# angela000/DQNFlappyBird

Measured on NVIDIA B200. Metric: env frames/sec (step+render+preproc), higher is better.
Workload: dtype u8

## Files before the change

dqnflappybird_b200/_lib.py:

```python
from __future__ import annotations

import ctypes as C
import glob
import os
import subprocess

_PKG = os.path.dirname(os.path.abspath(__file__))
_CSRC = os.path.join(_PKG, "csrc")
SO_PATH = os.path.join(_PKG, "libflappy_b200.so")

NVCC_FLAGS = [
    "-gencode", "arch=compute_100a,code=sm_100a", "-lineinfo", "-O3", "-std=c++17",
    "-Xcompiler", "-fPIC", "-shared",
]


class FlappyError(RuntimeError):
    pass


def sources():
    return sorted(glob.glob(os.path.join(_CSRC, "*.cu")))


# ... 117 lines not shown
    "fb_replay_sample_uniform": ([_vp, C.c_longlong, C.c_int, C.c_uint32, C.c_uint64, _i32p, _vp], C.c_int),
    "fb_replay_gather": ([_vp, _u8p, _u8p, _f32p, _u8p, C.c_longlong, C.c_int, _i32p, C.c_int, _u8p, _u8p, _f32p, _u8p, _i32p, _i32p, _vp], C.c_int),
    "fb_per_store": ([_vp, C.c_longlong, C.c_int, _vp], C.c_int),
    "fb_per_sample": ([_vp, C.c_int, C.c_double, C.c_uint64, _i32p, _i32p, _vp, _vp, _f32p, _vp], C.c_int),
    "fb_per_update": ([_vp, _i32p, _f32p, _vp, C.c_int, C.c_int, _vp], C.c_int),
    "fb_per_tree_copy": ([_vp, _vp, C.c_int, _vp], C.c_int),
    "fb_per_aux_tree_copy": ([_vp, C.c_int, _vp, C.c_int, _vp], C.c_int),
    "fb_per_min_root": ([_vp, _vp, _vp], C.c_int),
    "fb_per_set_global_min": ([_vp, _vp], C.c_int),
    "fb_replay_rng_pos": ([_vp, _vp, C.c_int, _vp], C.c_int),
    "fb_debug_assets_load_host": ([C.c_char_p, C.c_size_t], C.c_int),
    "fb_debug_host_reset": ([_i32p, _u8p, C.c_int, C.c_uint64, C.c_uint64], C.c_int),
    "fb_debug_host_step": ([_i32p, C.c_int, _u8p, C.c_int, C.c_uint64, C.c_uint64, _f32p, _u8p, _i32p], C.c_int),
    "fb_debug_host_obs": ([_i32p, C.c_int, _u8p], C.c_int),
    "fb_debug_host_mixed": ([_i32p], C.c_int),
    "fb_debug_tc_mma_rate": ([C.c_int, C.c_int, C.c_int, C.c_int, C.c_int, _vp, _vp], C.c_int),
    "fb_debug_tc_kernel": ([_vp, C.c_int, C.c_int, C.c_int, _f32p, _vp], C.c_int),
    "fb_debug_tc_slab": ([C.c_int, C.c_int, _vp, _vp, _f32p, _vp], C.c_int),
    "fb_debug_tc_gemm": ([C.c_int, C.c_int, C.c_int, C.c_int, C.c_int, _vp, _vp, _f32p, _vp, _vp], C.c_int),
}


def declared_symbols():
    return sorted(_SIGNATURES)


def lib():
    global _lib
    if _lib is None:
        if needs_build():
            build()
# ... 30 lines not shown
```

dqnflappybird_b200/csrc/fb_qnet_tc.cu:

```cuda
#include <cudaTypedefs.h>

#include <stdlib.h>
#include <string.h>

#include <map>
#include <new>
#include <vector>

#include "fb_qnet.cuh"
#include "fb_pack.cuh"
#include "fb_tc.cuh"
#include "fb_tc_conv.cuh"


namespace {

constexpr int kStages = 4;
constexpr int kMaxKb = 32;
constexpr int kG1 = 21, kP1 = 441;
constexpr int kG2 = 7, kP2 = 49;
constexpr int kThreads = 192;

struct GemmParams {
    int nkb, kper;
// ... 1328 lines not shown
    int n_sms;
    cudaStream_t aux;
    cudaStream_t aux2;
    cudaStream_t aux4;
    cudaStream_t aux3;
    cudaStream_t cap;
    cudaEvent_t ev[16];
    std::vector<GraphEntry> graphs;
    int use_graph;
    int f16;
    int fuse_fwd;
    int nopdl;
    int fuse_bwd;
    int step_samples;
    int conv1_mode;
};

namespace {

constexpr int kChunk1 = 1024, kChunk23 = 256;
constexpr int kFc1Splits = 5;
constexpr int kFuseMaxBatch = 512;
bool fused_head_ok(const QnetLayout &L) { return L.hidden == 512; }
int head_ctas(const TcState *t, int B) { const int c = (B + 3) / 4, m = t->n_sms < kMaxHeadCtas ? t->n_sms : kMaxHeadCtas; return c < m ? c : m; }

constexpr int kSlab1 = 152, kSlab2 = 136, kSlab3 = 144;
constexpr int kSlabW1 = 88, kSlabW2 = 72, kSlabW3 = 88;

int plan_splits(long long P, int target, int *klen_out) {
    if (target < 1) target = 1;
// ... 135 lines not shown
    FB_CUDA_OK(cudaDeviceGetAttribute(&t->n_sms, cudaDevAttrMultiProcessorCount, dev));
    {
        int lo = 0, hi = 0;
        FB_CUDA_OK(cudaDeviceGetStreamPriorityRange(&lo, &hi));
        FB_CUDA_OK(cudaStreamCreateWithPriority(&t->aux, cudaStreamNonBlocking, lo));
        FB_CUDA_OK(cudaStreamCreateWithPriority(&t->aux2, cudaStreamNonBlocking, hi));
        FB_CUDA_OK(cudaStreamCreateWithPriority(&t->aux3, cudaStreamNonBlocking, hi));
        FB_CUDA_OK(cudaStreamCreateWithPriority(&t->aux4, cudaStreamNonBlocking, lo));
        FB_CUDA_OK(cudaStreamCreateWithPriority(&t->cap, cudaStreamNonBlocking, hi));
    }
    for (auto &e : t->ev) FB_CUDA_OK(cudaEventCreateWithFlags(&e, cudaEventDisableTiming));
    t->use_graph = 1;
    { const char *e = getenv("FB_TC_FUSE_BWD"); t->fuse_bwd = (e && e[0] == '0') ? 0 : 1; }
    { const char *e = getenv("FB_TC_FUSE_FWD"); t->fuse_fwd = (e && e[0] == '0') ? 0 : 1; }
    { const char *e = getenv("FB_TC_CONV1_MODE"); t->conv1_mode = (e && e[0] >= '0' && e[0] <= '4') ? e[0] - '0' : 4; }
    { const char *e = getenv("FB_TC_NOPDL"); t->nopdl = e ? atoi(e) : 1; }
    n->tc = t;
    return FB_OK;
}

void tc_state_destroy(fb_qnet *n) {
    TcState *t = n->tc;
    if (!t) return;
    for (auto &g : t->graphs) destroy_entry(g);
    for (int w = 0; w < 2; w++) {
        FwdWs &f = t->ws[w];
        void *fs[] = {f.x2, f.z1, f.p2, f.a2, f.a3, f.parth, f.h1};
        for (void *p : fs) cudaFree(p);
    }
    void *ps[] = {t->dh1, t->dz3, t->dz2, t->dp2, t->dz1, t->part1, t->part2, t->part3, t->bp1, t->bp2, t->bp3, t->hp, t->hb, t->loss_terms,
// ... 81 lines not shown
    const QnetLayout &L = n->L;
    const TcWeightMaps &wm = t->wm[slot];
    const FwdWs &f = t->ws[w];
    const int P1 = B * kP1, P2 = B * kP2;
    g_probe_view = fv;
    const int c1mode = conv1_mode_at(t, B);
    if (c1mode == 0) {
        FB_CUDA_OK(tc::launch_pdl(pack_x2_kernel, dim3((unsigned)(((size_t)P1 * 8 + 255) / 256)), dim3(256), 0, st, fv, B, f.x2, t->f16));
        FB_CUDA_OK((launch_tc_conv<32, kSlab1, 1, 4, 6, 1>(p->x2_s[w], wm.w1p, p->conv1, t->n_sms, EpiConv1{f.z1, params_dev + L.b1, P1, t->f16}, st)));
        FB_CUDA_OK(tc::launch_pdl(pool_pack_kernel, dim3((unsigned)(((size_t)B * 36 * 16 + 255) / 256)), dim3(256), 0, st, f.z1, B, f.p2, t->f16));
    } else if ((keep && c1mode != 3) || c1mode == 1) {
        FB_CUDA_OK(tc::launch_pdl(pack_x2_kernel, dim3((unsigned)(((size_t)P1 * 8 + 255) / 256)), dim3(256), 0, st, fv, B, f.x2, t->f16));
        FB_CUDA_OK((launch_tc_conv1_fused<6, true>(p->x2_s[w], wm.w1p, Conv1FusedParams{fv, B, params_dev + L.b1, keep ? f.z1 : nullptr, f.p2, t->f16},
                                                  t->n_sms, st)));
    } else {
        FB_CUDA_OK((launch_tc_conv1_fused<4, false>(p->x2_s[w], wm.w1p, Conv1FusedParams{fv, B, params_dev + L.b1, keep ? f.z1 : nullptr, f.p2, t->f16}, t->n_sms, st)));
    }
    if (t->fuse_fwd && B <= kFuseMaxBatch) {
        FB_CUDA_OK((launch_tc_fwd23<2>(p->p2_s[w], wm.w2p, wm.w3p, Fwd23Params{(B + 1) / 2, B, params_dev + L.b2, params_dev + L.b3, keep ? f.a2 : nullptr, f.a3, t->f16},
                                       t->n_sms, st)));
    } else {
        FB_CUDA_OK((launch_tc_conv<64, kSlab2, 2, 8, 3, 1>(p->p2_s[w], wm.w2p, p->conv2, t->n_sms, EpiGrid7{f.a2, params_dev + L.b2, P2, t->f16}, st)));
        FB_CUDA_OK((launch_tc_conv<64, kSlab3, 1, 9, 4, 1>(p->a2_s[w], wm.w3p, p->conv3, t->n_sms, EpiConv3{f.a3, params_dev + L.b3, P2, t->f16}, st)));
    }
    FB_CUDA_OK((launch_tc_gemm<128, 2>(p->a3_k[w], wm.wf1n, p->fc1, dim3((B + 127) / 128, L.hidden / 128, p->sf),
                                       EpiStoreF32{f.parth, B, L.hidden, (size_t)n->max_batch * L.hidden}, st)));
    if (join) FB_CUDA_OK(cudaStreamWaitEvent(st, join, 0));
    TdFuse none{};
    if (td != nullptr && ap != nullptr && fused_head_ok(L))
        FB_CUDA_OK(tc::launch_pdl(fc1_head_train_kernel<16>, dim3(head_ctas(t, B)), dim3(128), 0, st, f.parth, p->sf,
                                  (size_t)n->max_batch * L.hidden, params_dev, L, B, q_out, *td, HeadBwd{t->dh1, t->hp, t->hb, GradFmt{t->f16, gscale}}, *ap));
// ... 320 lines not shown
    for (int r = 0; r < reps; r++) {
        switch (which) {
            case 0: FB_CUDA_OK((launch_tc_conv<32, kSlab1, 1, 4, 6, 1>(p->x2_s[0], wm.w1p, p->conv1, t->n_sms, EpiConv1{f.z1, params_dev + L.b1, P1, t->f16}, st))); break;
            case 1: FB_CUDA_OK((launch_tc_conv<64, kSlab2, 2, 8, 3, 1>(p->p2_s[0], wm.w2p, p->conv2, t->n_sms, EpiGrid7{f.a2, params_dev + L.b2, P2, t->f16}, st))); break;
            case 2: FB_CUDA_OK((launch_tc_conv<64, kSlab3, 1, 9, 4, 1>(p->a2_s[0], wm.w3p, p->conv3, t->n_sms, EpiConv3{f.a3, params_dev + L.b3, P2, t->f16}, st))); break;
            case 3: FB_CUDA_OK((launch_tc_gemm<128, 2>(p->a3_k[0], wm.wf1n, p->fc1, dim3((B + 127) / 128, H / 128, p->sf),
                                                       EpiStoreF32{f.parth, B, H, (size_t)n->max_batch * H}, st))); break;
            case 4: FB_CUDA_OK((launch_tc_wgrad<32, 2, kSlabW1, 1, 6>(p->x2_w, p->dz1_b, p->conv1_w, p->s1, EpiStoreF32{t->part1, 256, 32, (size_t)256 * 32}, st))); break;
            case 5: FB_CUDA_OK((launch_tc_conv<64, kSlab3, 1, 9, 4, 1>(p->dz3_s, wm.w3d, p->conv3_d, t->n_sms, EpiConv3Dgrad{t->dz2, f.a2, P2, t->f16}, st))); break;
            case 6: FB_CUDA_OK((launch_tc_gemm<64, 0>(p->dh1_k, wm.wf1n, p->fc1_d, dim3((B + 127) / 128, kFlat / 64, 1), EpiFc1Dgrad{t->dz3, f.a3, B, t->f16}, st))); break;
            case 7: FB_CUDA_OK((launch_tc_conv1_fused<4, false>(p->x2_s[0], wm.w1p, Conv1FusedParams{g_probe_view, B, params_dev + L.b1, nullptr, f.p2, t->f16}, t->n_sms, st))); break;
            case 8: FB_CUDA_OK((launch_tc_conv1_fused<4, false>(p->x2_s[0], wm.w1p, Conv1FusedParams{g_probe_view, B, params_dev + L.b1, f.z1, f.p2, t->f16}, t->n_sms, st))); break;
            case 9: FB_CUDA_OK((launch_tc_conv1_fused<6, true>(p->x2_s[0], wm.w1p, Conv1FusedParams{g_probe_view, B, params_dev + L.b1, nullptr, f.p2, t->f16}, t->n_sms, st))); break;
            case 10: FB_CUDA_OK((launch_tc_conv1_fused<6, true>(p->x2_s[0], wm.w1p, Conv1FusedParams{g_probe_view, B, params_dev + L.b1, f.z1, f.p2, t->f16}, t->n_sms, st))); break;
            case 11: FB_CUDA_OK((launch_tc_conv1_fused<6, true>(p->x2_s[0], wm.w1p, Conv1FusedParams{g_probe_view, B, params_dev + L.b1, nullptr, nullptr, t->f16}, t->n_sms, st))); break;
            default: FB_REQUIRE(false, "fb_debug_tc_kernel: which must be 0..11");
        }
    }
    return FB_OK;
}

namespace {
__global__ void __launch_bounds__(128) tc_slab_probe_kernel(const __grid_constant__ CUtensorMap mapA, const __grid_constant__ CUtensorMap mapB,
                                                            int shift, uint32_t base_offset, float *d) {
    extern __shared__ uint8_t smem_raw[];
    __shared__ __align__(8) uint64_t bar_full, bar_done;
    __shared__ uint32_t tmem_slot;
    const uint32_t smem = (tc::smem_u32(smem_raw) + 1023u) & ~1023u;
    const int warp = threadIdx.x >> 5, lane = threadIdx.x & 31;
    if (threadIdx.x == 0) { tc::mbar_init(tc::smem_u32(&bar_full), 1); tc::mbar_init(tc::smem_u32(&bar_done), 1); tc::fence_barrier_init(); }
    if (warp == 0) tc::tmem_alloc(tc::smem_u32(&tmem_slot), 64);
// ... 28 lines not shown

extern "C" int fb_debug_tc_slab(int shift, int base_offset, const void *a_dev, const void *b_dev, float *d_dev, void *stream) {
    FB_REQUIRE(a_dev && b_dev && d_dev && shift >= 0 && shift <= 128, "fb_debug_tc_slab: bad argument");
    int rc = ensure_encode();
    if (rc) return rc;
    CUtensorMap ma, mb;
    if ((rc = make_map(&ma, (const bf16 *)a_dev, 256, 64, 64, 128))) return rc;
    if ((rc = make_map(&mb, (const bf16 *)b_dev, 64, 64, 64, 64))) return rc;
    FB_CUDA_OK(cudaFuncSetAttribute(tc_slab_probe_kernel, cudaFuncAttributeMaxDynamicSharedMemorySize, 32768 + 8192 + 1024));
    tc_slab_probe_kernel<<<1, 128, 32768 + 8192 + 1024, (cudaStream_t)stream>>>(ma, mb, shift, (uint32_t)base_offset, d_dev);
    FB_CUDA_OK(cudaGetLastError());
    return FB_OK;
}

namespace {
__global__ void __launch_bounds__(128) tc_mma_rate_kernel(int n, int mn_major, int naccs, int iters, int same_operands, long long *cycles) {
    extern __shared__ uint8_t smem_raw[];
    __shared__ __align__(8) uint64_t bar;
    __shared__ uint32_t tmem_slot;
    const uint32_t smem = (tc::smem_u32(smem_raw) + 1023u) & ~1023u;
    const int warp = threadIdx.x >> 5;
    for (int i = threadIdx.x; i < 48 * 1024 / 4; i += 128) reinterpret_cast<uint32_t *>(smem_raw)[i] = 0x3c003c00u;
    if (threadIdx.x == 0) { tc::mbar_init(tc::smem_u32(&bar), 1); tc::fence_barrier_init(); }
    if (warp == 0) tc::tmem_alloc(tc::smem_u32(&tmem_slot), 512);
    tc::fence_proxy_async();
    tc::tc_fence_before(); __syncthreads(); tc::tc_fence_after();
    const uint32_t tmem = tmem_slot;
    if (warp == 1) {
        const uint32_t idesc = tc::instr_desc_bf16(128, n, mn_major, mn_major);
        const uint32_t hi = tc::smem_desc_hi(1024, tc::kSwizzle128);
        const uint32_t a0 = tc::smem_desc_lo(smem, mn_major ? 8192 : 16), b0 = tc::smem_desc_lo(smem + 16384, mn_major ? 8192 : 16);
        const uint32_t step = same_operands ? 0 : (mn_major ? 128 : 2);
        const uint32_t d1 = naccs > 1 ? (uint32_t)n : 0, d2 = naccs > 2 ? 2u * n : 0, d3 = naccs > 3 ? 3u * n : d1;
        uint32_t elected;
        asm volatile("{\n\t.reg .pred p;\n\telect.sync _|p, 0xffffffff;\n\tselp.b32 %0, 1, 0, p;\n\t}" : "=r"(elected));
        long long t0 = clock64();
        for (int i = 0; i < iters; i += 8) {
            if (elected) {
                tc::umma_bf16_lohi(tmem, a0, hi, b0, hi, idesc, 1);
                tc::umma_bf16_lohi(tmem + d1, a0 + step, hi, b0 + step, hi, idesc, 1);
                tc::umma_bf16_lohi(tmem + d2, a0 + 2 * step, hi, b0 + 2 * step, hi, idesc, 1);
                tc::umma_bf16_lohi(tmem + d3, a0 + 3 * step, hi, b0 + 3 * step, hi, idesc, 1);
                tc::umma_bf16_lohi(tmem, a0, hi, b0, hi, idesc, 1);
// ... 3 lines not shown
            }
            __syncwarp();
        }
        long long t_issue = clock64();
        if (elected) tc::umma_commit(tc::smem_u32(&bar));
        __syncwarp();
        tc::mbar_wait(tc::smem_u32(&bar), 0);
        long long t1 = clock64();
        if (elected) { cycles[0] = t1 - t0; cycles[1] = t_issue - t0; }
    }
    tc::tc_fence_before(); __syncthreads();
    if (warp == 0) tc::tmem_dealloc(tmem, 512);
}
}

extern "C" int fb_debug_tc_mma_rate(int n, int mn_major, int naccs, int iters, int same_operands, long long *cycles_dev, void *stream) {
    FB_REQUIRE(cycles_dev && n >= 16 && n <= 256 && n % 16 == 0 && naccs >= 1 && naccs * n <= 512 && iters > 0, "fb_debug_tc_mma_rate: bad argument");
    FB_CUDA_OK(cudaFuncSetAttribute(tc_mma_rate_kernel, cudaFuncAttributeMaxDynamicSharedMemorySize, 64 * 1024));
    tc_mma_rate_kernel<<<1, 128, 64 * 1024, (cudaStream_t)stream>>>(n, mn_major, naccs, iters, same_operands, cycles_dev);
    FB_CUDA_OK(cudaGetLastError());
    return FB_OK;
}

extern "C" int fb_debug_tc_gemm(int mode, int bn, int M, int N, int K, const void *a_dev, const void *b_dev, float *d_dev,
                                const uint32_t *strides6, void *stream) {
    FB_REQUIRE(a_dev && b_dev && d_dev && (mode == 0 || mode == 1) && (bn == 32 || bn == 64 || bn == 128) && N % bn == 0,
               "fb_debug_tc_gemm: bad argument");
    int rc = ensure_encode();
    if (rc) return rc;
    cudaStream_t st = (cudaStream_t)stream;
    CUtensorMap ma, mb;
    GemmParams g{};
    const bf16 *A = (const bf16 *)a_dev, *Bm = (const bf16 *)b_dev;
    dim3 grid;
// ... 26 lines not shown
```

dqnflappybird_b200/csrc/fb_tc.cuh:

```cuda
#pragma once
#include <cuda.h>
#include <cuda_bf16.h>
#include <cuda_fp16.h>
#include <cuda_runtime.h>
#include <stdint.h>

namespace tc {

__device__ __forceinline__ uint32_t smem_u32(const void *p) { return (uint32_t)__cvta_generic_to_shared(p); }

__device__ __forceinline__ bool elect_one() {
    uint32_t e;
    asm volatile("{\n\t.reg .pred p;\n\telect.sync _|p, 0xffffffff;\n\tselp.b32 %0, 1, 0, p;\n\t}" : "=r"(e));
    return e != 0;
}

__device__ __forceinline__ void mbar_init(uint32_t bar, uint32_t count) {
    asm volatile("mbarrier.init.shared::cta.b64 [%0], %1;" ::"r"(bar), "r"(count));
}
__device__ __forceinline__ void fence_barrier_init() { asm volatile("fence.mbarrier_init.release.cluster;" ::: "memory"); }
__device__ __forceinline__ void fence_proxy_async() { asm volatile("fence.proxy.async.shared::cta;" ::: "memory"); }
__device__ __forceinline__ void mbar_arrive(uint32_t bar) {
    asm volatile("mbarrier.arrive.shared::cta.b64 _, [%0];" ::"r"(bar) : "memory");
}
// ... 50 lines not shown
        "{\n\t.reg .pred p;\n\t"
        "setp.ne.b32 p, %4, 0;\n\t"
        "tcgen05.mma.cta_group::1.kind::f16 [%0], %1, %2, %3, p;\n\t}"
        ::"r"(d_tmem), "l"(adesc), "l"(bdesc), "r"(idesc), "r"(accumulate)
        : "memory");
}
__device__ __forceinline__ void umma_bf16_lohi(uint32_t d_tmem, uint32_t alo, uint32_t ahi, uint32_t blo, uint32_t bhi, uint32_t idesc,
                                               uint32_t accumulate) {
    asm volatile(
        "{\n\t.reg .pred p;\n\t.reg .b64 da, db;\n\t"
        "mov.b64 da, {%1, %2};\n\t"
        "mov.b64 db, {%3, %4};\n\t"
        "setp.ne.b32 p, %6, 0;\n\t"
        "tcgen05.mma.cta_group::1.kind::f16 [%0], da, db, %5, p;\n\t}"
        ::"r"(d_tmem), "r"(alo), "r"(ahi), "r"(blo), "r"(bhi), "r"(idesc), "r"(accumulate)
        : "memory");
}
__device__ __forceinline__ void umma_commit(uint32_t bar) {
    asm volatile("tcgen05.commit.cta_group::1.mbarrier::arrive::one.shared::cluster.b64 [%0];" ::"r"(bar) : "memory");
}
__device__ __forceinline__ void tmem_ld16(uint32_t taddr, float (&v)[16]) {
    uint32_t r[16];
    asm volatile(
        "tcgen05.ld.sync.aligned.32x32b.x16.b32 {%0,%1,%2,%3,%4,%5,%6,%7,%8,%9,%10,%11,%12,%13,%14,%15}, [%16];"
        : "=r"(r[0]), "=r"(r[1]), "=r"(r[2]), "=r"(r[3]), "=r"(r[4]), "=r"(r[5]), "=r"(r[6]), "=r"(r[7]), "=r"(r[8]),
          "=r"(r[9]), "=r"(r[10]), "=r"(r[11]), "=r"(r[12]), "=r"(r[13]), "=r"(r[14]), "=r"(r[15])
        : "r"(taddr));
    asm volatile("tcgen05.wait::ld.sync.aligned;" ::: "memory");
#pragma unroll
    for (int i = 0; i < 16; i++) v[i] = __uint_as_float(r[i]);
// ... 1 lines not shown

__device__ __forceinline__ void tmem_ld32(uint32_t taddr, float (&v)[32]) {
    uint32_t r[32];
    asm volatile(
        "tcgen05.ld.sync.aligned.32x32b.x32.b32 "
        "{%0,%1,%2,%3,%4,%5,%6,%7,%8,%9,%10,%11,%12,%13,%14,%15,%16,%17,%18,%19,%20,%21,%22,%23,%24,%25,%26,%27,%28,%29,%30,%31}, [%32];"
        : "=r"(r[0]), "=r"(r[1]), "=r"(r[2]), "=r"(r[3]), "=r"(r[4]), "=r"(r[5]), "=r"(r[6]), "=r"(r[7]), "=r"(r[8]), "=r"(r[9]),
          "=r"(r[10]), "=r"(r[11]), "=r"(r[12]), "=r"(r[13]), "=r"(r[14]), "=r"(r[15]), "=r"(r[16]), "=r"(r[17]), "=r"(r[18]), "=r"(r[19]),
          "=r"(r[20]), "=r"(r[21]), "=r"(r[22]), "=r"(r[23]), "=r"(r[24]), "=r"(r[25]), "=r"(r[26]), "=r"(r[27]), "=r"(r[28]), "=r"(r[29]),
          "=r"(r[30]), "=r"(r[31])
        : "r"(taddr));
    asm volatile("tcgen05.wait::ld.sync.aligned;" ::: "memory");
#pragma unroll
    for (int i = 0; i < 32; i++) v[i] = __uint_as_float(r[i]);
}

enum : uint32_t { kSwizzle128 = 2, kSwizzle64 = 4 };
__host__ __device__ constexpr uint64_t smem_desc(uint32_t addr, uint32_t lbo_bytes, uint32_t sbo_bytes, uint32_t layout) {
    return (uint64_t)((addr >> 4) & 0x3FFFu) | ((uint64_t)((lbo_bytes >> 4) & 0x3FFFu) << 16) |
           ((uint64_t)((sbo_bytes >> 4) & 0x3FFFu) << 32) | (1ull << 46) | ((uint64_t)layout << 61);
}
__host__ __device__ constexpr uint32_t smem_desc_lo(uint32_t addr, uint32_t lbo_bytes) {
    return ((addr >> 4) & 0x3FFFu) | (((lbo_bytes >> 4) & 0x3FFFu) << 16);
}
__host__ __device__ constexpr uint32_t smem_desc_hi(uint32_t sbo_bytes, uint32_t layout) {
    return ((sbo_bytes >> 4) & 0x3FFFu) | (1u << 14) | (layout << 29);
}
__host__ __device__ constexpr uint32_t instr_desc_bf16(int m, int n, int a_mn_major, int b_mn_major) {
    return (1u << 4) | (1u << 7) | (1u << 10) | ((uint32_t)a_mn_major << 15) | ((uint32_t)b_mn_major << 16) |
           ((uint32_t)(n >> 3) << 17) | ((uint32_t)(m >> 4) << 24);
// ... 60 lines not shown
```

dqnflappybird_b200/csrc/fb_tc_conv.cuh:

```cuda
#pragma once
#include "fb_tc.cuh"

namespace {

constexpr int kConvThreads = 192;

constexpr size_t kExclusiveSmem = 116 * 1024;
constexpr size_t exclusive_smem(size_t need) { return need > kExclusiveSmem ? need : kExclusiveSmem; }

struct ConvParams {
    int n_tiles;
    int slab_row0;
    int kb_rowoff[16];
    int kb_half[16];
    int f16;
};

template <int BN, int SLAB_ROWS, int NHALF, int NKB, int S, int T, class EP>
__global__ void __launch_bounds__(kConvThreads, 1) tc_conv_kernel(const __grid_constant__ CUtensorMap mapA,
                                                                   const __grid_constant__ CUtensorMap mapB, const ConvParams g, const EP ep) {
    constexpr uint32_t HALF_BYTES = SLAB_ROWS * 128, STAGE = NHALF * HALF_BYTES, BBLK = BN * 128, B_BYTES = NKB * BBLK;
    static_assert(SLAB_ROWS % 8 == 0 && SLAB_ROWS <= 256, "slab rows: multiple of 8 (1024-byte stage alignment), one TMA box");
    static_assert(S % T == 0 && 2 * T * BN <= 512, "a group of T tiles occupies T consecutive stages and T accumulators of a set");
    extern __shared__ uint8_t smem_raw[];
// ... 299 lines not shown
#pragma unroll
    for (int k = 0; k < K; k++) {
        const bool valid = (dst[k] & 0x80000000u) != 0;
        uint32_t w[4];
#pragma unroll
        for (int s2 = 0; s2 < 2; s2++)
#pragma unroll
            for (int h = 0; h < 2; h++) {
                const float lo = (float)((t[k][2 * h] >> (8 * s2)) & 255), hi = (float)((t[k][2 * h + 1] >> (8 * s2)) & 255);
                w[s2 * 2 + h] = valid ? tc::pack2(lo, hi, f16) : 0u;
            }
        if (tid + k * NT <= LAST) *reinterpret_cast<uint4 *>(slab + (dst[k] & 0x7fffffffu)) = make_uint4(w[0], w[1], w[2], w[3]);
    }
}

struct Conv1FusedParams {
    FrameView fv;
    int B;
    const float *bias;
    __nv_bfloat16 *z1;
    __nv_bfloat16 *p2;
    int f16;
};

template <int S, bool FROM_X2>
__global__ void __launch_bounds__(FROM_X2 ? kRoleThreads1 : kFusedThreads, 1) tc_conv1_fused_kernel(const __grid_constant__ CUtensorMap mapA,
                                                                                          const __grid_constant__ CUtensorMap mapB,
                                                                                          const Conv1FusedParams g) {
    constexpr int BN = 32, NKB = 4;
    constexpr uint32_t STAGE = kSlabF * 128, BBLK = BN * 128, B_BYTES = NKB * BBLK, ZS_BYTES = 128 * BN * 2;
    extern __shared__ uint8_t smem_raw[];
    __shared__ __align__(8) uint64_t bar_full[S], bar_empty[S], bar_b, bar_acc_full[2], bar_acc_empty[2], bar_raw_full[kRawStages],
        bar_raw_empty[kRawStages];
    __shared__ uint32_t tmem_slot;
    __shared__ __align__(16) float bias_s[BN];
    uint8_t *smem_gen = smem_raw + ((1024u - (tc::smem_u32(smem_raw) & 1023u)) & 1023u);
    const uint32_t smem_b = tc::smem_u32(smem_gen), smem_a = smem_b + B_BYTES;
    uint8_t *slab_gen = smem_gen + B_BYTES, *zs_gen = slab_gen + S * STAGE, *raw_gen = zs_gen + 4 * ZS_BYTES;
    const int warp = threadIdx.x >> 5, lane = threadIdx.x & 31;
    const int n_tiles = 4 * g.B;
    const long long total_rows = (long long)g.B * 441;

    if (threadIdx.x == 0) {
        tc::tma_prefetch_desc(&mapB);
        for (int s = 0; s < S; s++) { tc::mbar_init(tc::smem_u32(&bar_full[s]), 1); tc::mbar_init(tc::smem_u32(&bar_empty[s]), 1); }
        tc::mbar_init(tc::smem_u32(&bar_b), 1);
        for (int a = 0; a < 2; a++) { tc::mbar_init(tc::smem_u32(&bar_acc_full[a]), 1); tc::mbar_init(tc::smem_u32(&bar_acc_empty[a]), 4); }
        for (int k = 0; k < kRawStages; k++) { tc::mbar_init(tc::smem_u32(&bar_raw_full[k]), 1); tc::mbar_init(tc::smem_u32(&bar_raw_empty[k]), 1); }
        tc::fence_barrier_init();
    }
    if (warp == 1) tc::tmem_alloc(tc::smem_u32(&tmem_slot), 64);
    tc::tc_fence_before();
    __syncthreads();
    tc::tc_fence_after();
    const uint32_t tmem = tmem_slot;
    if (threadIdx.x == 0) {
        tc::mbar_expect_tx(tc::smem_u32(&bar_b), B_BYTES);
        for (int kb = 0; kb < NKB; kb++) tc::tma_load_2d(smem_b + kb * BBLK, &mapB, kb * 64, 0, tc::smem_u32(&bar_b));
    }
    if (threadIdx.x >= 64 && threadIdx.x < 64 + BN) bias_s[threadIdx.x - 64] = g.bias[threadIdx.x - 64];
    tc::pdl_wait();
    tc::pdl_launch();
    __syncthreads();

    if (warp == 0 && FROM_X2) {
        const bool leader = tc::elect_one();
// ... 11 lines not shown
    } else if (warp == 0) {
        const bool leader = tc::elect_one();
        int i = 0;
        for (int tile = blockIdx.x; tile < n_tiles; tile += gridDim.x, i++) {
            const int rs = i % kRawStages, b = tile >> 2, tq = tile & 3;
            tc::mbar_wait(tc::smem_u32(&bar_raw_empty[rs]), ((i / kRawStages) & 1) ^ 1u);
            if (leader) {
                const int ih0 = 24 * tq - 2, lo = ih0 < 0 ? 0 : ih0, hi = ih0 + kRawRows > 80 ? 80 : ih0 + kRawRows;
                const uint32_t bytes = (uint32_t)(hi - lo) * 80u, full = tc::smem_u32(&bar_raw_full[rs]);
                const uint32_t dst = tc::smem_u32(raw_gen) + rs * kRawBytes + (uint32_t)(lo - ih0) * 80u;
                tc::mbar_expect_tx(full, 4 * bytes);
#pragma unroll
                for (int c = 0; c < 4; c++) tc::bulk_load_1d(dst + c * (kRawRows * 80), g.fv.chan(b, c) + lo * 80, bytes, full);
            }
            __syncwarp();
        }
    } else if (warp >= kRoleThreads1 / 32) {
        constexpr int GT = kBuilders / 2;
        const int grp = (threadIdx.x - kRoleThreads1) / GT, tid = (threadIdx.x - kRoleThreads1) - grp * GT;
        int i = grp;
        for (int tile = blockIdx.x + grp * (int)gridDim.x; tile < n_tiles; tile += 2 * (int)gridDim.x, i += 2) {
            const int s = i % S, rs = i % kRawStages;
            tc::mbar_wait(tc::smem_u32(&bar_raw_full[rs]), (i / kRawStages) & 1);
            tc::mbar_wait(tc::smem_u32(&bar_empty[s]), ((i / S) & 1) ^ 1u);
            slab_from_raw<GT>(slab_gen + s * STAGE, raw_gen + rs * kRawBytes, tile & 3, tid, g.f16);
            tc::fence_proxy_async();
            if (grp == 0) asm volatile("bar.sync 2, %0;" ::"n"(GT) : "memory");
            else asm volatile("bar.sync 3, %0;" ::"n"(GT) : "memory");
            if (tid == 0) { tc::mbar_arrive(tc::smem_u32(&bar_full[s])); tc::mbar_arrive(tc::smem_u32(&bar_raw_empty[rs])); }
        }
    } else if (warp == 1) {
        const bool leader = tc::elect_one();
        const uint32_t idesc = tc::instr_desc_16(128, BN, 0, 0, g.f16);
        constexpr uint32_t dhi = tc::smem_desc_hi(1024, tc::kSwizzle128);
        const uint32_t a_lo0 = tc::smem_desc_lo(smem_a, 16), b_lo0 = tc::smem_desc_lo(smem_b, 16);
        tc::mbar_wait(tc::smem_u32(&bar_b), 0);
        int i = 0;
        for (int tile = blockIdx.x; tile < n_tiles; tile += gridDim.x, i++) {
            const int s = i % S, as = i & 1;
            tc::mbar_wait(tc::smem_u32(&bar_acc_empty[as]), ((i >> 1) & 1) ^ 1u);
            tc::mbar_wait(tc::smem_u32(&bar_full[s]), (i / S) & 1);
            tc::tc_fence_after();
            if (leader) {
                const uint32_t a_lo = a_lo0 + s * (STAGE >> 4);
#pragma unroll
                for (int kb = 0; kb < NKB; kb++) {
                    const uint32_t tap = (uint32_t)(((kb >> 1) * 21 + (kb & 1)) * 128) >> 4;
#pragma unroll
                    for (int k = 0; k < 4; k++)
                        tc::umma_bf16_lohi(tmem + as * BN, a_lo + tap + 2 * k, dhi, b_lo0 + ((kb * BBLK + k * 32) >> 4), dhi, idesc, (kb | k) != 0);
                }
                tc::umma_commit(tc::smem_u32(&bar_empty[s]));
                tc::umma_commit(tc::smem_u32(&bar_acc_full[as]));
            }
            __syncwarp();
        }
    } else if (warp >= 2 && warp < kRoleThreads1 / 32) {
        const int eg = (warp - 2) >> 2;
// ... 45 lines not shown
                    const int r0 = (2 * ph_l) * 21 + 2 * pw;
                    uint4 m = ld(r0), o1 = ld(r0 + 1), o2 = ld(r0 + 21), o3 = ld(r0 + 22);
                    uint32_t *pm = reinterpret_cast<uint32_t *>(&m);
                    const uint32_t *p1 = reinterpret_cast<const uint32_t *>(&o1), *p2 = reinterpret_cast<const uint32_t *>(&o2),
                                   *p3 = reinterpret_cast<const uint32_t *>(&o3);
#pragma unroll
                    for (int k = 0; k < 4; k++) pm[k] = tc::max2(tc::max2(pm[k], p1[k], g.f16), tc::max2(p2[k], p3[k], g.f16), g.f16);
                    const int bh = (ph + 1) >> 1, rr = (ph + 1) & 1, bw = (pw + 1) >> 1, ss = (pw + 1) & 1;
                    *reinterpret_cast<uint4 *>(g.p2 + ((size_t)b * 49 + bh * 7 + bw) * 128 + rr * 64 + ss * 32 + cg * 8) = m;
                }
            }
        }
    }
    tc::tc_fence_before();
    __syncthreads();
    if (warp == 1) tc::tmem_dealloc(tmem, 64);
}

template <int S, bool FROM_X2>
static cudaError_t launch_tc_conv1_fused(const CUtensorMap &ma, const CUtensorMap &mb, const Conv1FusedParams &g, int max_ctas, cudaStream_t st) {
    static bool configured = false;
    auto kern = tc_conv1_fused_kernel<S, FROM_X2>;
    constexpr size_t smem = exclusive_smem(4 * 32 * 128 + (size_t)S * kSlabF * 128 + 4 * 128 * 32 * 2 + (FROM_X2 ? 0 : kRawStages * kRawBytes) + 1024);
    if (!configured) {
        cudaError_t e = cudaFuncSetAttribute(kern, cudaFuncAttributeMaxDynamicSharedMemorySize, (int)smem);
        if (e != cudaSuccess) return e;
        configured = true;
    }
    int grid = 4 * g.B < max_ctas ? 4 * g.B : max_ctas;
    return tc::launch_pdl(kern, dim3(grid), dim3(FROM_X2 ? kRoleThreads1 : kFusedThreads), smem, st, ma, mb, g);
}

}
```

include/flappy_b200.h:

```cpp
#ifndef FLAPPY_B200_H
#define FLAPPY_B200_H

#include <stddef.h>
#include <stdint.h>

#ifdef __cplusplus
extern "C" {
#endif

#define FB_OBS 80
#define FB_FRAME_BYTES 6400
#define FB_SCREEN_W 288
#define FB_SCREEN_H 512
#define FB_STATE_INTS 16

typedef enum {
    FB_OK = 0,
    FB_ERR_INVALID = -1,
    FB_ERR_CUDA = -2,
    FB_ERR_ASSETS = -3,
    FB_ERR_ACTION = -4,
    FB_ERR_STATE = -5
} fb_status;

// ... 144 lines not shown
                               const float *target_params_dev, const int32_t *chan_off_s_host4, const int32_t *chan_off_next_host4,
                               int global_batch, double gamma, int loss_sum, float *grads_dev, float *loss_out_dev,
                               float *abs_err_out_dev, float *q_target_out_dev, float *m_dev, float *v_dev, float lr, float beta1,
                               float beta2, float eps, float grad_scale, float beta1_power, float beta2_power, void *stream);


int fb_debug_assets_load_host(const uint8_t *packed_host, size_t n);
int fb_debug_step_sampling_layout(int32_t *out, int capacity);
int fb_debug_host_reset(int32_t *state16, const uint8_t *gaps, int gaps_len, uint64_t seed, uint64_t env_id);
int fb_debug_host_step(int32_t *state16, int action, const uint8_t *gaps, int gaps_len, uint64_t seed,
                       uint64_t env_id, float *reward, uint8_t *terminal, int32_t *score);
int fb_debug_host_obs(const int32_t *state16, int mode , uint8_t *out6400);
int fb_debug_host_mixed(const int32_t *state16);
int fb_debug_tc_gemm(int mode, int bn, int M, int N, int K, const void *a_bf16_dev, const void *b_bf16_dev, float *d_dev,
                     const uint32_t *strides6_host, void *stream);
int fb_debug_tc_mma_rate(int n, int mn_major, int naccs, int iters, int same_operands, long long *cycles_dev, void *stream);
int fb_debug_tc_kernel(fb_qnet *net, int which, int batch, int reps, const float *params_dev, void *stream);
int fb_debug_tc_slab(int shift, int base_offset, const void *a_bf16_dev, const void *b_bf16_dev, float *d_dev, void *stream);

#ifdef __cplusplus
}
#endif
#endif
```

Before: 846.1 million.

## Stage conv1 im2col A operand in tensor memory instead of shared memory

Adds a conv1 fused-kernel variant where builder warps write the im2col A tile straight into tensor memory with tcgen05.st, and the MMA issuer reads A from TMEM. This removes the shared-memory slab for A and the smem writes and reads on that path, at the cost of allocating all 512 TMEM columns and cutting to two pipeline stages. It is on by default in the raw-u8 conv1 mode and can be turned off with an env var. A microbenchmark option for the TMEM-A MMA rate is also added.

```diff
diff --git a/dqnflappybird_b200/_lib.py b/dqnflappybird_b200/_lib.py
--- a/dqnflappybird_b200/_lib.py
+++ b/dqnflappybird_b200/_lib.py
@@ -155,7 +155,7 @@
     "fb_debug_host_step": ([_i32p, C.c_int, _u8p, C.c_int, C.c_uint64, C.c_uint64, _f32p, _u8p, _i32p], C.c_int),
     "fb_debug_host_obs": ([_i32p, C.c_int, _u8p], C.c_int),
     "fb_debug_host_mixed": ([_i32p], C.c_int),
-    "fb_debug_tc_mma_rate": ([C.c_int, C.c_int, C.c_int, C.c_int, C.c_int, _vp, _vp], C.c_int),
+    "fb_debug_tc_mma_rate": ([C.c_int, C.c_int, C.c_int, C.c_int, C.c_int, C.c_int, _vp, _vp], C.c_int),
     "fb_debug_tc_kernel": ([_vp, C.c_int, C.c_int, C.c_int, _f32p, _vp], C.c_int),
     "fb_debug_tc_slab": ([C.c_int, C.c_int, _vp, _vp, _f32p, _vp], C.c_int),
     "fb_debug_tc_gemm": ([C.c_int, C.c_int, C.c_int, C.c_int, C.c_int, _vp, _vp, _f32p, _vp, _vp], C.c_int),
diff --git a/dqnflappybird_b200/csrc/fb_qnet_tc.cu b/dqnflappybird_b200/csrc/fb_qnet_tc.cu
--- a/dqnflappybird_b200/csrc/fb_qnet_tc.cu
+++ b/dqnflappybird_b200/csrc/fb_qnet_tc.cu
@@ -1366,6 +1366,7 @@
     int fuse_bwd;
     int step_samples;
     int conv1_mode;
+    int conv1_tmem;
 };
 
 namespace {
@@ -1531,6 +1532,7 @@
     { const char *e = getenv("FB_TC_FUSE_BWD"); t->fuse_bwd = (e && e[0] == '0') ? 0 : 1; }
     { const char *e = getenv("FB_TC_FUSE_FWD"); t->fuse_fwd = (e && e[0] == '0') ? 0 : 1; }
     { const char *e = getenv("FB_TC_CONV1_MODE"); t->conv1_mode = (e && e[0] >= '0' && e[0] <= '4') ? e[0] - '0' : 4; }
+    { const char *e = getenv("FB_TC_CONV1_TMEM"); t->conv1_tmem = (e && e[0] == '0') ? 0 : 1; }
     { const char *e = getenv("FB_TC_NOPDL"); t->nopdl = e ? atoi(e) : 1; }
     n->tc = t;
     return FB_OK;
@@ -1642,7 +1644,9 @@
         FB_CUDA_OK((launch_tc_conv1_fused<6, true>(p->x2_s[w], wm.w1p, Conv1FusedParams{fv, B, params_dev + L.b1, keep ? f.z1 : nullptr, f.p2, t->f16},
                                                   t->n_sms, st)));
     } else {
-        FB_CUDA_OK((launch_tc_conv1_fused<4, false>(p->x2_s[w], wm.w1p, Conv1FusedParams{fv, B, params_dev + L.b1, keep ? f.z1 : nullptr, f.p2, t->f16}, t->n_sms, st)));
+        const Conv1FusedParams c1{fv, B, params_dev + L.b1, keep ? f.z1 : nullptr, f.p2, t->f16};
+        if (t->conv1_tmem) FB_CUDA_OK((launch_tc_conv1_fused<2, false, true>(p->x2_s[w], wm.w1p, c1, t->n_sms, st)));
+        else FB_CUDA_OK((launch_tc_conv1_fused<4, false>(p->x2_s[w], wm.w1p, c1, t->n_sms, st)));
     }
     if (t->fuse_fwd && B <= kFuseMaxBatch) {
         FB_CUDA_OK((launch_tc_fwd23<2>(p->p2_s[w], wm.w2p, wm.w3p, Fwd23Params{(B + 1) / 2, B, params_dev + L.b2, params_dev + L.b3, keep ? f.a2 : nullptr, f.a3, t->f16},
@@ -1993,7 +1997,9 @@
             case 9: FB_CUDA_OK((launch_tc_conv1_fused<6, true>(p->x2_s[0], wm.w1p, Conv1FusedParams{g_probe_view, B, params_dev + L.b1, nullptr, f.p2, t->f16}, t->n_sms, st))); break;
             case 10: FB_CUDA_OK((launch_tc_conv1_fused<6, true>(p->x2_s[0], wm.w1p, Conv1FusedParams{g_probe_view, B, params_dev + L.b1, f.z1, f.p2, t->f16}, t->n_sms, st))); break;
             case 11: FB_CUDA_OK((launch_tc_conv1_fused<6, true>(p->x2_s[0], wm.w1p, Conv1FusedParams{g_probe_view, B, params_dev + L.b1, nullptr, nullptr, t->f16}, t->n_sms, st))); break;
-            default: FB_REQUIRE(false, "fb_debug_tc_kernel: which must be 0..11");
+            case 12: FB_CUDA_OK((launch_tc_conv1_fused<2, false, true>(p->x2_s[0], wm.w1p, Conv1FusedParams{g_probe_view, B, params_dev + L.b1, nullptr, f.p2, t->f16}, t->n_sms, st))); break;
+            case 13: FB_CUDA_OK((launch_tc_conv1_fused<2, false, true>(p->x2_s[0], wm.w1p, Conv1FusedParams{g_probe_view, B, params_dev + L.b1, f.z1, f.p2, t->f16}, t->n_sms, st))); break;
+            default: FB_REQUIRE(false, "fb_debug_tc_kernel: which must be 0..13");
         }
     }
     return FB_OK;
@@ -2052,7 +2058,8 @@
 }
 
 namespace {
-__global__ void __launch_bounds__(128) tc_mma_rate_kernel(int n, int mn_major, int naccs, int iters, int same_operands, long long *cycles) {
+__global__ void __launch_bounds__(128) tc_mma_rate_kernel(int n, int mn_major, int naccs, int iters, int same_operands, int a_tmem,
+                                                          long long *cycles) {
     extern __shared__ uint8_t smem_raw[];
     __shared__ __align__(8) uint64_t bar;
     __shared__ uint32_t tmem_slot;
@@ -2063,8 +2070,41 @@
     if (warp == 0) tc::tmem_alloc(tc::smem_u32(&tmem_slot), 512);
     tc::fence_proxy_async();
     tc::tc_fence_before(); __syncthreads(); tc::tc_fence_after();
-    const uint32_t tmem = tmem_slot;
-    if (warp == 1) {
+    const uint32_t tmem = tmem_slot, ta = tmem + 480;
+    if (a_tmem) {
+        const uint32_t r[8] = {0x3c003c00u, 0x3c003c00u, 0x3c003c00u, 0x3c003c00u, 0x3c003c00u, 0x3c003c00u, 0x3c003c00u, 0x3c003c00u};
+        for (int c = 0; c < 32; c += 8) tc::tmem_st8(ta + ((uint32_t)(warp * 32) << 16) + (uint32_t)c, r);
+        tc::tmem_st_wait();
+        tc::tc_fence_before(); __syncthreads(); tc::tc_fence_after();
+    }
+    if (warp == 1 && a_tmem) {
+        const uint32_t idesc = tc::instr_desc_bf16(128, n, 0, mn_major);
+        const uint32_t hi = tc::smem_desc_hi(1024, tc::kSwizzle128);
+        const uint32_t b0 = tc::smem_desc_lo(smem + 16384, mn_major ? 8192 : 16);
+        const uint32_t step = same_operands ? 0 : (mn_major ? 128 : 2), astep = same_operands ? 0 : 8;
+        const uint32_t d1 = naccs > 1 ? (uint32_t)n : 0, d2 = naccs > 2 ? 2u * n : 0, d3 = naccs > 3 ? 3u * n : d1;
+        const bool elected = tc::elect_one();
+        long long t0 = clock64();
+        for (int i = 0; i < iters; i += 8) {
+            if (elected) {
+                tc::umma_tmem_a(tmem, ta, b0, hi, idesc, 1);
+                tc::umma_tmem_a(tmem + d1, ta + astep, b0 + step, hi, idesc, 1);
+                tc::umma_tmem_a(tmem + d2, ta + 2 * astep, b0 + 2 * step, hi, idesc, 1);
+                tc::umma_tmem_a(tmem + d3, ta + 3 * astep, b0 + 3 * step, hi, idesc, 1);
+                tc::umma_tmem_a(tmem, ta, b0, hi, idesc, 1);
+                tc::umma_tmem_a(tmem + d1, ta + astep, b0 + step, hi, idesc, 1);
+                tc::umma_tmem_a(tmem + d2, ta + 2 * astep, b0 + 2 * step, hi, idesc, 1);
+                tc::umma_tmem_a(tmem + d3, ta + 3 * astep, b0 + 3 * step, hi, idesc, 1);
+            }
+            __syncwarp();
+        }
+        long long t_issue = clock64();
+        if (elected) tc::umma_commit(tc::smem_u32(&bar));
+        __syncwarp();
+        tc::mbar_wait(tc::smem_u32(&bar), 0);
+        long long t1 = clock64();
+        if (elected) { cycles[0] = t1 - t0; cycles[1] = t_issue - t0; }
+    } else if (warp == 1) {
         const uint32_t idesc = tc::instr_desc_bf16(128, n, mn_major, mn_major);
         const uint32_t hi = tc::smem_desc_hi(1024, tc::kSwizzle128);
         const uint32_t a0 = tc::smem_desc_lo(smem, mn_major ? 8192 : 16), b0 = tc::smem_desc_lo(smem + 16384, mn_major ? 8192 : 16);
@@ -2098,10 +2138,12 @@
 }
 }
 
-extern "C" int fb_debug_tc_mma_rate(int n, int mn_major, int naccs, int iters, int same_operands, long long *cycles_dev, void *stream) {
-    FB_REQUIRE(cycles_dev && n >= 16 && n <= 256 && n % 16 == 0 && naccs >= 1 && naccs * n <= 512 && iters > 0, "fb_debug_tc_mma_rate: bad argument");
+extern "C" int fb_debug_tc_mma_rate(int n, int mn_major, int naccs, int iters, int same_operands, int a_tmem, long long *cycles_dev,
+                                    void *stream) {
+    FB_REQUIRE(cycles_dev && n >= 16 && n <= 256 && n % 16 == 0 && naccs >= 1 && naccs * n <= (a_tmem ? 480 : 512) && iters > 0,
+               "fb_debug_tc_mma_rate: bad argument");
     FB_CUDA_OK(cudaFuncSetAttribute(tc_mma_rate_kernel, cudaFuncAttributeMaxDynamicSharedMemorySize, 64 * 1024));
-    tc_mma_rate_kernel<<<1, 128, 64 * 1024, (cudaStream_t)stream>>>(n, mn_major, naccs, iters, same_operands, cycles_dev);
+    tc_mma_rate_kernel<<<1, 128, 64 * 1024, (cudaStream_t)stream>>>(n, mn_major, naccs, iters, same_operands, a_tmem ? 1 : 0, cycles_dev);
     FB_CUDA_OK(cudaGetLastError());
     return FB_OK;
 }
diff --git a/dqnflappybird_b200/csrc/fb_tc.cuh b/dqnflappybird_b200/csrc/fb_tc.cuh
--- a/dqnflappybird_b200/csrc/fb_tc.cuh
+++ b/dqnflappybird_b200/csrc/fb_tc.cuh
@@ -88,6 +88,15 @@
         "setp.ne.b32 p, %6, 0;\n\t"
         "tcgen05.mma.cta_group::1.kind::f16 [%0], da, db, %5, p;\n\t}"
         ::"r"(d_tmem), "r"(alo), "r"(ahi), "r"(blo), "r"(bhi), "r"(idesc), "r"(accumulate)
+        : "memory");
+}
+__device__ __forceinline__ void umma_tmem_a(uint32_t d_tmem, uint32_t a_tmem, uint32_t blo, uint32_t bhi, uint32_t idesc, uint32_t accumulate) {
+    asm volatile(
+        "{\n\t.reg .pred p;\n\t.reg .b64 db;\n\t"
+        "mov.b64 db, {%2, %3};\n\t"
+        "setp.ne.b32 p, %5, 0;\n\t"
+        "tcgen05.mma.cta_group::1.kind::f16 [%0], [%1], db, %4, p;\n\t}"
+        ::"r"(d_tmem), "r"(a_tmem), "r"(blo), "r"(bhi), "r"(idesc), "r"(accumulate)
         : "memory");
 }
 __device__ __forceinline__ void umma_commit(uint32_t bar) {
@@ -119,6 +128,12 @@
 #pragma unroll
     for (int i = 0; i < 32; i++) v[i] = __uint_as_float(r[i]);
 }
+
+__device__ __forceinline__ void tmem_st8(uint32_t taddr, const uint32_t (&r)[8]) {
+    asm volatile("tcgen05.st.sync.aligned.32x32b.x8.b32 [%0], {%1,%2,%3,%4,%5,%6,%7,%8};"
+                 ::"r"(taddr), "r"(r[0]), "r"(r[1]), "r"(r[2]), "r"(r[3]), "r"(r[4]), "r"(r[5]), "r"(r[6]), "r"(r[7]));
+}
+__device__ __forceinline__ void tmem_st_wait() { asm volatile("tcgen05.wait::st.sync.aligned;" ::: "memory"); }
 
 enum : uint32_t { kSwizzle128 = 2, kSwizzle64 = 4 };
 __host__ __device__ constexpr uint64_t smem_desc(uint32_t addr, uint32_t lbo_bytes, uint32_t sbo_bytes, uint32_t layout) {
diff --git a/dqnflappybird_b200/csrc/fb_tc_conv.cuh b/dqnflappybird_b200/csrc/fb_tc_conv.cuh
--- a/dqnflappybird_b200/csrc/fb_tc_conv.cuh
+++ b/dqnflappybird_b200/csrc/fb_tc_conv.cuh
@@ -337,6 +337,62 @@
     }
 }
 
+template <bool F16>
+__device__ __forceinline__ void cvt_u8x2_pair(uint32_t x, uint32_t y, int s, uint32_t &w0, uint32_t &w1) {
+    if (F16) {
+        const uint32_t t = __byte_perm(x, y, (uint32_t)(s | ((4 + s) << 4) | ((s + 1) << 8) | ((5 + s) << 12)));
+        const __half2 k = __halves2half2(__ushort_as_half((unsigned short)0xE400), __ushort_as_half((unsigned short)0xE400));
+        uint32_t a = __byte_perm(t, 0x64646464u, 0x4140), b = __byte_perm(t, 0x64646464u, 0x4342);
+        __half2 ha = __hadd2(*reinterpret_cast<__half2 *>(&a), k), hb = __hadd2(*reinterpret_cast<__half2 *>(&b), k);
+        w0 = *reinterpret_cast<uint32_t *>(&ha); w1 = *reinterpret_cast<uint32_t *>(&hb);
+    } else {
+        w0 = tc::pack2((float)((x >> (8 * s)) & 255), (float)((y >> (8 * s)) & 255), 0);
+        w1 = tc::pack2((float)((x >> (8 * s + 8)) & 255), (float)((y >> (8 * s + 8)) & 255), 0);
+    }
+}
+
+template <bool F16>
+__device__ __forceinline__ void tmem_row_from_raw(uint32_t ta, const uint8_t *raw, int tq, int r) {
+    const int bh_l = (r * 3121) >> 16, bw = r - bh_l * 21;
+    const uint32_t *rw = reinterpret_cast<const uint32_t *>(raw);
+    const bool okA = bw >= 1, okB = bw <= 19, okC = bw <= 18;
+    const int wA = okA ? bw - 1 : 0, wB = okB ? bw : 0, wC = okC ? bw + 1 : 0;
+#pragma unroll
+    for (int y0 = 0; y0 < 8; y0 += 4) {
+        uint32_t a[4][4], b[4][4], c[4][4];
+#pragma unroll
+        for (int y = 0; y < 4; y++) {
+            const int rr = 4 * bh_l + y0 + y, ih = 24 * tq - 2 + rr;
+            const bool rok = (unsigned)ih < 80u;
+#pragma unroll
+            for (int f = 0; f < 4; f++) {
+                const uint32_t *row = rw + f * (kRawRows * 20) + rr * 20;
+                const uint32_t va = row[wA], vb = row[wB], vc = row[wC];
+                a[y][f] = rok && okA ? va : 0u;
+                b[y][f] = rok && okB ? vb : 0u;
+                c[y][f] = rok && okC ? vc : 0u;
+            }
+        }
+#pragma unroll
+        for (int y = 0; y < 4; y++) {
+            uint32_t lo[4], hi[4];
+#pragma unroll
+            for (int f = 0; f < 4; f++) { lo[f] = __funnelshift_r(a[y][f], b[y][f], 16); hi[f] = __funnelshift_r(b[y][f], c[y][f], 16); }
+            uint32_t w0[8], w1[8];
+#pragma unroll
+            for (int s = 0; s < 4; s += 2)
+#pragma unroll
+                for (int cp = 0; cp < 2; cp++) {
+                    cvt_u8x2_pair<F16>(lo[2 * cp], lo[2 * cp + 1], s, w0[s * 2 + cp], w0[s * 2 + 2 + cp]);
+                    cvt_u8x2_pair<F16>(hi[2 * cp], hi[2 * cp + 1], s, w1[s * 2 + cp], w1[s * 2 + 2 + cp]);
+                }
+            const int dr = (y0 + y) >> 2, k = (y0 + y) & 3;
+            tc::tmem_st8(ta + (uint32_t)(((2 * dr) * 4 + k) * 8), w0);
+            tc::tmem_st8(ta + (uint32_t)(((2 * dr + 1) * 4 + k) * 8), w1);
+        }
+    }
+}
+
 struct Conv1FusedParams {
     FrameView fv;
     int B;
@@ -346,12 +402,15 @@
     int f16;
 };
 
-template <int S, bool FROM_X2>
+constexpr uint32_t kATmemCol = 64;
+template <int S, bool FROM_X2, bool A_TMEM = false>
 __global__ void __launch_bounds__(FROM_X2 ? kRoleThreads1 : kFusedThreads, 1) tc_conv1_fused_kernel(const __grid_constant__ CUtensorMap mapA,
                                                                                           const __grid_constant__ CUtensorMap mapB,
                                                                                           const Conv1FusedParams g) {
     constexpr int BN = 32, NKB = 4;
     constexpr uint32_t STAGE = kSlabF * 128, BBLK = BN * 128, B_BYTES = NKB * BBLK, ZS_BYTES = 128 * BN * 2;
+    constexpr uint32_t SLAB_BYTES = A_TMEM ? 0 : S * STAGE, TMEM_COLS = A_TMEM ? 512 : 64;
+    static_assert(!A_TMEM || (S == 2 && !FROM_X2 && kATmemCol + S * 128 <= TMEM_COLS), "A_TMEM: two stages of 128 columns, u8 builders");
     extern __shared__ uint8_t smem_raw[];
     __shared__ __align__(8) uint64_t bar_full[S], bar_empty[S], bar_b, bar_acc_full[2], bar_acc_empty[2], bar_raw_full[kRawStages],
         bar_raw_empty[kRawStages];
@@ -359,20 +418,20 @@
     __shared__ __align__(16) float bias_s[BN];
     uint8_t *smem_gen = smem_raw + ((1024u - (tc::smem_u32(smem_raw) & 1023u)) & 1023u);
     const uint32_t smem_b = tc::smem_u32(smem_gen), smem_a = smem_b + B_BYTES;
-    uint8_t *slab_gen = smem_gen + B_BYTES, *zs_gen = slab_gen + S * STAGE, *raw_gen = zs_gen + 4 * ZS_BYTES;
+    uint8_t *slab_gen = smem_gen + B_BYTES, *zs_gen = slab_gen + SLAB_BYTES, *raw_gen = zs_gen + 4 * ZS_BYTES;
     const int warp = threadIdx.x >> 5, lane = threadIdx.x & 31;
     const int n_tiles = 4 * g.B;
     const long long total_rows = (long long)g.B * 441;
 
     if (threadIdx.x == 0) {
         tc::tma_prefetch_desc(&mapB);
-        for (int s = 0; s < S; s++) { tc::mbar_init(tc::smem_u32(&bar_full[s]), 1); tc::mbar_init(tc::smem_u32(&bar_empty[s]), 1); }
+        for (int s = 0; s < S; s++) { tc::mbar_init(tc::smem_u32(&bar_full[s]), A_TMEM ? 4 : 1); tc::mbar_init(tc::smem_u32(&bar_empty[s]), 1); }
         tc::mbar_init(tc::smem_u32(&bar_b), 1);
         for (int a = 0; a < 2; a++) { tc::mbar_init(tc::smem_u32(&bar_acc_full[a]), 1); tc::mbar_init(tc::smem_u32(&bar_acc_empty[a]), 4); }
-        for (int k = 0; k < kRawStages; k++) { tc::mbar_init(tc::smem_u32(&bar_raw_full[k]), 1); tc::mbar_init(tc::smem_u32(&bar_raw_empty[k]), 1); }
+        for (int k = 0; k < kRawStages; k++) { tc::mbar_init(tc::smem_u32(&bar_raw_full[k]), 1); tc::mbar_init(tc::smem_u32(&bar_raw_empty[k]), A_TMEM ? 4 : 1); }
         tc::fence_barrier_init();
     }
-    if (warp == 1) tc::tmem_alloc(tc::smem_u32(&tmem_slot), 64);
+    if (warp == 1) tc::tmem_alloc(tc::smem_u32(&tmem_slot), TMEM_COLS);
     tc::tc_fence_before();
     __syncthreads();
     tc::tc_fence_after();
@@ -414,6 +473,23 @@
                 for (int c = 0; c < 4; c++) tc::bulk_load_1d(dst + c * (kRawRows * 80), g.fv.chan(b, c) + lo * 80, bytes, full);
             }
             __syncwarp();
+        }
+    } else if (A_TMEM && warp >= kRoleThreads1 / 32) {
+        constexpr int GT = kBuilders / 2;
+        const int grp = (threadIdx.x - kRoleThreads1) / GT, r = (warp & 3) * 32 + lane;
+        int i = grp;
+        for (int tile = blockIdx.x + grp * (int)gridDim.x; tile < n_tiles; tile += 2 * (int)gridDim.x, i += 2) {
+            const int s = i % S, rs = i % kRawStages;
+            tc::mbar_wait(tc::smem_u32(&bar_raw_full[rs]), (i / kRawStages) & 1);
+            tc::mbar_wait(tc::smem_u32(&bar_empty[s]), ((i / S) & 1) ^ 1u);
+            tc::tc_fence_after();
+            const uint32_t ta = tmem + ((uint32_t)((warp & 3) * 32) << 16) + kATmemCol + (uint32_t)s * 128;
+            if (g.f16) tmem_row_from_raw<true>(ta, raw_gen + rs * kRawBytes, tile & 3, r);
+            else tmem_row_from_raw<false>(ta, raw_gen + rs * kRawBytes, tile & 3, r);
+            tc::tmem_st_wait();
+            tc::tc_fence_before();
+            __syncwarp();
+            if (lane == 0) { tc::mbar_arrive(tc::smem_u32(&bar_full[s])); tc::mbar_arrive(tc::smem_u32(&bar_raw_empty[rs])); }
         }
     } else if (warp >= kRoleThreads1 / 32) {
         constexpr int GT = kBuilders / 2;
@@ -441,7 +517,16 @@
             tc::mbar_wait(tc::smem_u32(&bar_acc_empty[as]), ((i >> 1) & 1) ^ 1u);
             tc::mbar_wait(tc::smem_u32(&bar_full[s]), (i / S) & 1);
             tc::tc_fence_after();
-            if (leader) {
+            if (A_TMEM && leader) {
+                const uint32_t ta = tmem + kATmemCol + (uint32_t)s * 128;
+#pragma unroll
+                for (int kb = 0; kb < NKB; kb++)
+#pragma unroll
+                    for (int k = 0; k < 4; k++)
+                        tc::umma_tmem_a(tmem + as * BN, ta + (uint32_t)(kb * 4 + k) * 8, b_lo0 + ((kb * BBLK + k * 32) >> 4), dhi, idesc, (kb | k) != 0);
+                tc::umma_commit(tc::smem_u32(&bar_empty[s]));
+                tc::umma_commit(tc::smem_u32(&bar_acc_full[as]));
+            } else if (leader) {
                 const uint32_t a_lo = a_lo0 + s * (STAGE >> 4);
 #pragma unroll
                 for (int kb = 0; kb < NKB; kb++) {
@@ -517,14 +602,14 @@
     }
     tc::tc_fence_before();
     __syncthreads();
-    if (warp == 1) tc::tmem_dealloc(tmem, 64);
-}
-
-template <int S, bool FROM_X2>
+    if (warp == 1) tc::tmem_dealloc(tmem, TMEM_COLS);
+}
+
+template <int S, bool FROM_X2, bool A_TMEM = false>
 static cudaError_t launch_tc_conv1_fused(const CUtensorMap &ma, const CUtensorMap &mb, const Conv1FusedParams &g, int max_ctas, cudaStream_t st) {
     static bool configured = false;
-    auto kern = tc_conv1_fused_kernel<S, FROM_X2>;
-    constexpr size_t smem = exclusive_smem(4 * 32 * 128 + (size_t)S * kSlabF * 128 + 4 * 128 * 32 * 2 + (FROM_X2 ? 0 : kRawStages * kRawBytes) + 1024);
+    auto kern = tc_conv1_fused_kernel<S, FROM_X2, A_TMEM>;
+    constexpr size_t smem = exclusive_smem(4 * 32 * 128 + (A_TMEM ? 0 : (size_t)S * kSlabF * 128) + 4 * 128 * 32 * 2 + (FROM_X2 ? 0 : kRawStages * kRawBytes) + 1024);
     if (!configured) {
         cudaError_t e = cudaFuncSetAttribute(kern, cudaFuncAttributeMaxDynamicSharedMemorySize, (int)smem);
         if (e != cudaSuccess) return e;
diff --git a/include/flappy_b200.h b/include/flappy_b200.h
--- a/include/flappy_b200.h
+++ b/include/flappy_b200.h
@@ -182,7 +182,7 @@
 int fb_debug_host_mixed(const int32_t *state16);
 int fb_debug_tc_gemm(int mode, int bn, int M, int N, int K, const void *a_bf16_dev, const void *b_bf16_dev, float *d_dev,
                      const uint32_t *strides6_host, void *stream);
-int fb_debug_tc_mma_rate(int n, int mn_major, int naccs, int iters, int same_operands, long long *cycles_dev, void *stream);
+int fb_debug_tc_mma_rate(int n, int mn_major, int naccs, int iters, int same_operands, int a_tmem, long long *cycles_dev, void *stream);
 int fb_debug_tc_kernel(fb_qnet *net, int which, int batch, int reps, const float *params_dev, void *stream);
 int fb_debug_tc_slab(int shift, int base_offset, const void *a_bf16_dev, const void *b_bf16_dev, float *d_dev, void *stream);
 
```

Result: no change. 843.3 million (median of 6 runs) (-0.3%).
